# SonghuaHu-UMD/MultiSTGraph

Hardware: AMD Instinct MI355X
Metric: forward node-steps/s (B*T*N per second), MultiATGCN.predict (higher is better)
Workload: dtype f32; 1 GPU; Baltimore 403-node, in=24h out=24h, batch=64/GPU, multi+unidirection K=5; nodes=403, per_gpu_batch=64, global_batch=64, in_steps=24, out_steps=24, parallelism=batch shards, no data-path collective (dp1), layer_wavefront_streams=True

## Files before the change

multistgraph_amd/csrc/matgcn_kernels.hip:

```cpp
#include <hip/hip_runtime.h>
#include <stdint.h>

#include "matgcn_internal.h"

typedef __attribute__((ext_vector_type(16))) float f32x16;
typedef unsigned int u32x4 __attribute__((ext_vector_type(4)));
typedef __attribute__((ext_vector_type(4))) float f32x4;
#define MFMA16(a, b, c) __builtin_amdgcn_mfma_f32_16x16x4f32((a), (b), (c), 0, 0, 0)

#define MFMA32(a, b, c) __builtin_amdgcn_mfma_f32_32x32x2f32((a), (b), (c), 0, 0, 0)

__device__ __forceinline__ float sigmoid_f(float x) { return 1.0f / (1.0f + expf(-x)); }

__device__ __forceinline__ int acc_row(int r, int half) { return (r & 3) + 8 * (r >> 2) + 4 * half; }

__global__ __launch_bounds__(256) void k_adaptive_adj(const float* __restrict__ e1, const float* __restrict__ e2,
                                                      int rank, int bidir, int N, float* __restrict__ plain, int ldP) {
  extern __shared__ float logits[];
  __shared__ float red[256];
  __shared__ float erow[64];
  const int n = blockIdx.x, tid = threadIdx.x;
  for (int r = tid; r < rank; r += 256) erow[r] = e1[(size_t)n * rank + r];
  __syncthreads();
  float mx = 0.f;
// ... 16 lines not shown
  }
  mx = red[0];
  __syncthreads();
  float sum = 0.f;
  for (int m = tid; m < N; m += 256) {
    const float e = expf(logits[m] - mx);
    logits[m] = e;
    sum += e;
  }
  red[tid] = sum;
  __syncthreads();
  for (int s = 128; s > 0; s >>= 1) {
    if (tid < s) red[tid] += red[tid + s];
    __syncthreads();
  }
  const float inv = 1.0f / red[0];
  for (int m = tid; m < N; m += 256) plain[(size_t)n * ldP + m] = logits[m] * inv;
}

__global__ __launch_bounds__(256) void k_static_transpose(const float* __restrict__ S, int N, int ldSrc,
                                                          float* __restrict__ St, int ldS, int col0,
                                                          float* __restrict__ plain, int ldP, int accumulate) {
  __shared__ float tile[32][33];
  const int bx = blockIdx.x * 32, by = blockIdx.y * 32;
  const int tx = threadIdx.x & 31, ty = threadIdx.x >> 5;
  for (int j = ty; j < 32; j += 8) {
    const int n = by + j, m = bx + tx;
    const float v = (n < N && m < N) ? S[(size_t)n * ldSrc + m] : 0.f;
    tile[j][tx] = v;
    if (plain && plain != S && n < N && m < N) plain[(size_t)n * ldP + m] = v;
  }
  __syncthreads();
  for (int j = ty; j < 32; j += 8) {
    const int m = bx + j, n = by + tx;
    if (m < N && n < N) {
      float* dst = &St[(size_t)m * ldS + col0 + n];
      *dst = accumulate ? *dst + tile[tx][j] : tile[tx][j];
    }
  }
}

__global__ __launch_bounds__(256) void k_cheb_combine(const float* __restrict__ prod, const float* __restrict__ prev2,
                                                      int prev2_is_identity, int N, int ldP, float* __restrict__ St,
                                                      int ldS, int col0, float* __restrict__ plain_out) {
  __shared__ float tile[32][33];
  const int bx = blockIdx.x * 32, by = blockIdx.y * 32;
  const int tx = threadIdx.x & 31, ty = threadIdx.x >> 5;
  for (int j = ty; j < 32; j += 8) {
    const int n = by + j, m = bx + tx;
    float v = 0.f;
    if (n < N && m < N) {
      const float p2 = prev2_is_identity ? (n == m ? 1.f : 0.f) : prev2[(size_t)n * ldP + m];
      v = 2.0f * prod[(size_t)n * ldP + m] - p2;
      plain_out[(size_t)n * ldP + m] = v;
    }
    tile[j][tx] = v;
  }
  __syncthreads();
  for (int j = ty; j < 32; j += 8) {
    const int m = bx + j, n = by + tx;
    if (m < N && n < N) St[(size_t)m * ldS + col0 + n] = tile[tx][j];
  }
}

__global__ __launch_bounds__(256) void k_stack_tight(const float* __restrict__ St, int ldS, int Np, int N, int Ks,
                                                     float* __restrict__ tight, int ldT) {
  const size_t idx = (size_t)blockIdx.x * 256 + threadIdx.x;
  if (idx >= (size_t)Np * ldT) return;
  const int m = (int)(idx / ldT), c = (int)(idx % ldT);
  const int k = c / N, n = c - k * N;
  tight[idx] = k < Ks ? St[(size_t)m * ldS + k * Np + n] : 0.f;
}

__device__ __forceinline__ void stack_tail_zero(float* __restrict__ St, int ldS, float* __restrict__ StT, int ldT,
                                                int Np, int N, int Ks, int block, int nBlocks, int tid, int nThreads) {
  const int s0 = Ks * Np, t0 = Ks * N, ws = ldS - s0, wt = ldT - t0;
  for (int m = block; m < Np; m += nBlocks) {
    for (int c = tid; c < ws; c += nThreads) St[(size_t)m * ldS + s0 + c] = 0.f;
    for (int c = tid; c < wt; c += nThreads) StT[(size_t)m * ldT + t0 + c] = 0.f;
  }
}

template <int ROWS>
__global__ __launch_bounds__(256 * ROWS) void k_adaptive_stack(const float* __restrict__ e1, const float* __restrict__ e2,
                                                               int rank, int bidir, int N, int Np, int Ks,
                                                               float* __restrict__ St, int ldS, float* __restrict__ StT,
                                                               int ldT, int tail) {
  extern __shared__ float logitsAll[];
  __shared__ float redAll[ROWS][256];
  __shared__ float erowAll[ROWS][64];
  __shared__ float invAll[ROWS];
  const int sub = threadIdx.x >> 8, tid = threadIdx.x & 255;
  const int n0 = blockIdx.x * ROWS, n = n0 + sub;
  const bool live = n < N;
  float* logits = logitsAll + (size_t)sub * N;
  float* red = redAll[sub];
  float* erow = erowAll[sub];
  if (live)
    for (int r = tid; r < rank; r += 256) erow[r] = e1[(size_t)n * rank + r];
  __syncthreads();
  float mx = 0.f;
  if (live)
    for (int m = tid; m < N; m += 256) {
      float s = 0.f;
      if (bidir) {
        for (int r = 0; r < rank; ++r) s = fmaf(erow[r], e1[(size_t)m * rank + r], s);
      } else {
        for (int r = 0; r < rank; ++r) s = fmaf(erow[r], e2[(size_t)r * N + m], s);
      }
      s = fmaxf(s, 0.f);
      logits[m] = s;
      mx = fmaxf(mx, s);
    }
  red[tid] = mx;
  __syncthreads();
  for (int s = 128; s > 0; s >>= 1) {
    if (tid < s) red[tid] = fmaxf(red[tid], red[tid + s]);
    __syncthreads();
  }
  mx = red[0];
  __syncthreads();
  float sum = 0.f;
  if (live)
    for (int m = tid; m < N; m += 256) {
      const float e = expf(logits[m] - mx);
      logits[m] = e;
      sum += e;
    }
  red[tid] = sum;
  __syncthreads();
  for (int s = 128; s > 0; s >>= 1) {
    if (tid < s) red[tid] += red[tid + s];
    __syncthreads();
  }
  if (tid == 0) invAll[sub] = 1.0f / red[0];
  __syncthreads();
  for (int m = threadIdx.x; m < Np; m += 256 * ROWS) {
    float v[ROWS];
#pragma unroll
    for (int j = 0; j < ROWS; ++j) v[j] = (m < N && n0 + j < N) ? logitsAll[(size_t)j * N + m] * invAll[j] : 0.f;
    float* ds = St + (size_t)m * ldS + n0;
    float* dt = StT + (size_t)m * ldT + n0;
    if (ROWS == 4) {
      *reinterpret_cast<float4*>(ds) = make_float4(v[0], v[1], v[2], v[3]);
      if (n0 + 4 <= N) *reinterpret_cast<float4*>(dt) = make_float4(v[0], v[1], v[2], v[3]);
      else
#pragma unroll
        for (int j = 0; j < ROWS; ++j) if (n0 + j < N) dt[j] = v[j];
    } else {
#pragma unroll
      for (int j = 0; j < ROWS; ++j) {
        ds[j] = v[j];
        if (n0 + j < N) dt[j] = v[j];
      }
    }
  }
  if (tail) stack_tail_zero(St, ldS, StT, ldT, Np, N, Ks, blockIdx.x, gridDim.x, threadIdx.x, 256 * ROWS);
}

struct StaticStackArgs {
  const float* S[4];
  int slot[4];
};
__global__ __launch_bounds__(256) void k_static_stack(StaticStackArgs a, int N, int Np, int Ks, float* __restrict__ St,
                                                      int ldS, float* __restrict__ StT, int ldT, int tail) {
  __shared__ float tile[32][33];
  const float* __restrict__ S = a.S[blockIdx.z];
  const int slot = a.slot[blockIdx.z];
  const int bx = blockIdx.x * 32, by = blockIdx.y * 32;
  const int tx = threadIdx.x & 31, ty = threadIdx.x >> 5;
  for (int j = ty; j < 32; j += 8) {
    const int n = by + j, m = bx + tx;
    tile[j][tx] = (n < N && m < N) ? S[(size_t)n * N + m] : 0.f;
  }
  __syncthreads();
  for (int j = ty; j < 32; j += 8) {
    const int m = bx + j, n = by + tx;
    if (m < Np && n < Np) {
      St[(size_t)m * ldS + slot * Np + n] = tile[tx][j];
      if (n < N) StT[(size_t)m * ldT + slot * N + n] = tile[tx][j];
    }
  }
  if (tail)
    stack_tail_zero(St, ldS, StT, ldT, Np, N, Ks, (int)((blockIdx.z * gridDim.y + blockIdx.y) * gridDim.x + blockIdx.x),
                    (int)(gridDim.x * gridDim.y * gridDim.z), threadIdx.x, 256);
}

#define PREP_NB 8

__device__ __forceinline__ float cheb_scalar(float s, int order) {
  float t0 = 1.f, t1 = s;
  for (int j = 2; j <= order; ++j) { const float t2 = 2.f * s * t1 - t0; t0 = t1; t1 = t2; }
  return t1;
}

template <int KIND>
__global__ __launch_bounds__(256) void k_prep_stream(PrepStream a) {
  const int nBase = blockIdx.y * PREP_NB;
  const int unit = blockIdx.x * 256 + threadIdx.x;
  const int OT = a.O >> 4;
  if (unit >= a.groups * OT * 64) return;
  const int lane = unit & 63, ct = (unit >> 6) % OT, g = (unit >> 6) / OT;
  const int o = 16 * ct + (lane & 15);
  int slot[4], chan[4];
#pragma unroll
  for (int s = 0; s < 4; ++s) {
    if (KIND == 0) {
      const int kk = 16 * g + 4 * (lane >> 4) + s;
      slot[s] = kk >> 6; chan[s] = a.iOfs + (kk & 63);
    } else if (KIND == 1) {
      const int kk = 16 * g + 4 * (lane >> 4) + s;
      const int nx = a.map.nKeep * a.C0;
      if (kk < nx) { slot[s] = kk / a.C0; chan[s] = kk - slot[s] * a.C0; }
      else { slot[s] = kk == nx ? -2 : -1; chan[s] = 0; }
    }
  }
  float gmax = -3.0e38f, gsum = 1.f;
  if (a.wg) {
    gsum = 0.f;
    for (int k = 0; k < a.map.KtotOrig; ++k) gmax = fmaxf(gmax, a.wg[k]);
    for (int k = 0; k < a.map.KtotOrig; ++k) gsum += expf(a.wg[k] - gmax);
  }
  auto gk = [&](int k) { return a.wg ? expf(a.wg[k] - gmax) / gsum : 1.f; };
  const size_t dstride = (size_t)a.map.KtotOrig * a.I * a.O;
  float acc[PREP_NB][4];
#pragma unroll
  for (int b = 0; b < PREP_NB; ++b)
#pragma unroll
    for (int s = 0; s < 4; ++s) acc[b][s] = 0.f;
  size_t rofs[4];
  float scale[4];
#pragma unroll
  for (int s = 0; s < 4; ++s) {
    rofs[s] = 0; scale[s] = 0.f;
    if (slot[s] >= 0) {
      const int k = a.map.keepK[slot[s]];
      rofs[s] = ((size_t)k * a.I + chan[s]) * a.O + o;
      scale[s] = gk(k);
    } else if (slot[s] == -2) {
      scale[s] = 1.f;
    }
  }
#pragma unroll 4
  for (int dd = 0; dd < a.d; ++dd) {
    float pv[4];
#pragma unroll
    for (int s = 0; s < 4; ++s) {
      float v = 0.f;
      if (slot[s] >= 0) v = a.wpool[(size_t)dd * dstride + rofs[s]];
      else if (slot[s] == -2) v = a.bpool[(size_t)dd * a.O + o];
      pv[s] = v * scale[s];
    }
#pragma unroll
    for (int b = 0; b < PREP_NB; ++b) {
      const float e = a.E[(size_t)min(nBase + b, a.N - 1) * a.d + dd];
#pragma unroll
      for (int s = 0; s < 4; ++s) acc[b][s] = fmaf(e, pv[s], acc[b][s]);
    }
  }
  const bool anyIdent = slot[0] == 0 || slot[1] == 0 || slot[2] == 0 || slot[3] == 0;
  if (anyIdent) {
    for (int q = 0; q < a.map.nDiag; ++q) {
      const int k = a.map.diagK[q];
      const float gq = gk(k);
      float part[PREP_NB][4];
#pragma unroll
      for (int b = 0; b < PREP_NB; ++b)
#pragma unroll
        for (int s = 0; s < 4; ++s) part[b][s] = 0.f;
      for (int dd = 0; dd < a.d; ++dd) {
        float pv[4];
#pragma unroll
        for (int s = 0; s < 4; ++s)
          pv[s] = slot[s] == 0 ? a.wpool[(size_t)dd * dstride + ((size_t)k * a.I + chan[s]) * a.O + o] : 0.f;
#pragma unroll
        for (int b = 0; b < PREP_NB; ++b) {
          const float e = a.E[(size_t)min(nBase + b, a.N - 1) * a.d + dd];
#pragma unroll
          for (int s = 0; s < 4; ++s) part[b][s] = fmaf(e, pv[s], part[b][s]);
        }
      }
#pragma unroll
      for (int b = 0; b < PREP_NB; ++b) {
        const int n = min(nBase + b, a.N - 1);
        const float t = gq * cheb_scalar(a.map.diagSrc[q][(size_t)n * (a.map.N + 1)], a.map.diagOrder[q]);
#pragma unroll
        for (int s = 0; s < 4; ++s) acc[b][s] = fmaf(t, part[b][s], acc[b][s]);
      }
    }
  }
  size_t frag;
  if (a.OTdst > 0) frag = ((size_t)(g * a.OTdst + a.otOfs + ct) * 64 + lane) * 4;
  else frag = (size_t)unit * 4;
#pragma unroll
  for (int b = 0; b < PREP_NB; ++b) {
    const int n = nBase + b;
    if (n < a.N)
      *reinterpret_cast<float4*>(a.out + (size_t)n * a.nodeStride + a.baseOfs + frag) =
          make_float4(acc[b][0], acc[b][1], acc[b][2], acc[b][3]);
  }
}

template <int DS>
__global__ __launch_bounds__(256) void k_prep_mfma(PrepStream a, int tilesPerBlock) {
  const int tid = threadIdx.x, lane = tid & 63, w = tid >> 6;
  const int OT = a.O >> 4;
  const int pair = blockIdx.x >> 1, half = blockIdx.x & 1;
  const int ct = pair % OT, g = pair / OT;
  const int r = lane & 15, ka = lane >> 4;
  float gmax = -3.0e38f, gsum = 1.f;
  if (a.wg) {
    gsum = 0.f;
    for (int k = 0; k < a.map.KtotOrig; ++k) gmax = fmaxf(gmax, a.wg[k]);
    for (int k = 0; k < a.map.KtotOrig; ++k) gsum += expf(a.wg[k] - gmax);
  }
  auto gk = [&](int k) { return a.wg ? expf(a.wg[k] - gmax) / gsum : 1.f; };
  const size_t dstride = (size_t)a.map.KtotOrig * a.I * a.O;
  float A[8][DS], Aq[8][DS];
  bool ident = false;
#pragma unroll
  for (int q8 = 0; q8 < 8; ++q8) {
    const int kq = 2 * half + (q8 >> 2), j = 4 * (q8 & 3) + (r >> 2), sr = r & 3;
    const int o = 16 * ct + j;
    int slot, chan;
    if (g < a.groups) {
      const int kk = 16 * g + 4 * kq + sr;
      slot = kk >> 6; chan = a.iOfs + (kk & 63);
    } else {
      const int kk = 16 * (g - a.groups) + 4 * kq + sr;
      const int nx = a.map.nKeep * a.C0;
      if (kk < nx) { slot = kk / a.C0; chan = kk - slot * a.C0; }
      else { slot = kk == nx ? -2 : -1; chan = 0; }
    }
    const float* src = a.wpool; size_t sstep = 0; float scale = 0.f;
    if (slot >= 0) {
      const int k = a.map.keepK[slot];
      src = a.wpool + ((size_t)k * a.I + chan) * a.O + o; sstep = dstride; scale = gk(k);
    } else if (slot == -2) {
      src = a.bpool + o; sstep = (size_t)a.O; scale = 1.f;
    }
    const bool id = slot == 0 && a.map.nDiag > 0;
    ident = ident || id;
    const float* srcq = id ? a.wpool + ((size_t)a.map.diagK[0] * a.I + chan) * a.O + o : a.wpool;
#pragma unroll
    for (int st = 0; st < DS; ++st) {
      const int dd = 4 * st + ka;
      const float v = src[(size_t)min(dd, a.d - 1) * sstep];
      A[q8][st] = (dd < a.d && slot != -1) ? v * scale : 0.f;
      const float vq = srcq[(size_t)min(dd, a.d - 1) * (id ? dstride : 0)];
      Aq[q8][st] = (dd < a.d && id) ? vq : 0.f;
    }
  }
  const bool anyIdent = __ballot(ident) != 0ull;
  const int nTiles = (a.N + 15) >> 4;
  const int tile0 = blockIdx.y * tilesPerBlock, tile1 = min(tile0 + tilesPerBlock, nTiles);
  const int nodeL = lane & 15, kb = lane >> 4;
  auto load_b = [&](int tile, float (&Bf)[DS]) {
    const float* e = a.E + (size_t)min(tile * 16 + nodeL, a.N - 1) * a.d;
#pragma unroll
    for (int st = 0; st < DS; ++st) {
      const int dd = 4 * st + kb;
      const float v = e[min(dd, a.d - 1)];
      Bf[st] = dd < a.d ? v : 0.f;
    }
  };
  float Bf[DS], Bn[DS];
  if (tile0 + w < tile1) load_b(tile0 + w, Bf);
  for (int tile = tile0 + w; tile < tile1; tile += 4) {
    load_b(min(tile + 4, tile1 - 1), Bn);
    const int n = tile * 16 + nodeL;
    f32x4 acc[8];
#pragma unroll
    for (int q8 = 0; q8 < 8; ++q8) acc[q8] = f32x4{0.f, 0.f, 0.f, 0.f};
#pragma unroll
    for (int st = 0; st < DS; ++st)
#pragma unroll
      for (int q8 = 0; q8 < 8; ++q8) acc[q8] = MFMA16(A[q8][st], Bf[st], acc[q8]);
    if (anyIdent) {
      const int nc = min(n, a.N - 1);
      for (int q = 0; q < a.map.nDiag; ++q) {
        f32x4 part[8];
#pragma unroll
        for (int q8 = 0; q8 < 8; ++q8) part[q8] = f32x4{0.f, 0.f, 0.f, 0.f};
        if (q == 0) {
#pragma unroll
          for (int st = 0; st < DS; ++st)
#pragma unroll
            for (int q8 = 0; q8 < 8; ++q8) part[q8] = MFMA16(Aq[q8][st], Bf[st], part[q8]);
        } else {
          const int k = a.map.diagK[q];
#pragma unroll
          for (int q8 = 0; q8 < 8; ++q8) {
            const int kq = 2 * half + (q8 >> 2), j = 4 * (q8 & 3) + (r >> 2), sr = r & 3;
            int slot, chan;
            if (g < a.groups) { const int kk = 16 * g + 4 * kq + sr; slot = kk >> 6; chan = a.iOfs + (kk & 63); }
            else {
              const int kk = 16 * (g - a.groups) + 4 * kq + sr;
              if (kk < a.map.nKeep * a.C0) { slot = kk / a.C0; chan = kk - slot * a.C0; } else { slot = -1; chan = 0; }
            }
#pragma unroll
            for (int st = 0; st < DS; ++st) {
              const int dd = 4 * st + ka;
              const float v = a.wpool[(size_t)min(dd, a.d - 1) * dstride + ((size_t)k * a.I + chan) * a.O + 16 * ct + j];
              part[q8] = MFMA16((dd < a.d && slot == 0) ? v : 0.f, Bf[st], part[q8]);
            }
          }
        }
        const float t = gk(a.map.diagK[q]) *
                        cheb_scalar(a.map.diagSrc[q][(size_t)nc * (a.map.N + 1)], a.map.diagOrder[q]);
#pragma unroll
        for (int q8 = 0; q8 < 8; ++q8)
#pragma unroll
          for (int e = 0; e < 4; ++e) acc[q8][e] = fmaf(t, part[q8][e], acc[q8][e]);
      }
    }
    if (n < a.N) {
      float* dst = a.out + (size_t)n * a.nodeStride + a.baseOfs;
#pragma unroll
      for (int q8 = 0; q8 < 8; ++q8) {
        const int kq = 2 * half + (q8 >> 2), j = 4 * (q8 & 3) + kb;
        const size_t frag = ((size_t)(a.OTdst > 0 ? g * a.OTdst + a.otOfs + ct : g * OT + ct) * 64 + kq * 16 + j) * 4;
        *reinterpret_cast<float4*>(dst + frag) = make_float4(acc[q8][0], acc[q8][1], acc[q8][2], acc[q8][3]);
      }
    }
#pragma unroll
    for (int st = 0; st < DS; ++st) Bf[st] = Bn[st];
  }
}

__global__ __launch_bounds__(256) void k_prep_bias(const float* __restrict__ E, const float* __restrict__ bpool, int d,
                                                   int O, int N, float* __restrict__ out, int ldo, int colOfs) {
  const int idx = blockIdx.x * 256 + threadIdx.x;
  if (idx >= N * O) return;
  const int n = idx / O, o = idx - n * O;
  float s = 0.f;
  for (int dd = 0; dd < d; ++dd) s = fmaf(E[(size_t)n * d + dd], bpool[(size_t)dd * O + o], s);
  out[(size_t)n * ldo + colOfs + o] = s;
}

__device__ __forceinline__ void prep_linear(const float* __restrict__ W, int I, int O, int C, int Cpad, int rows, int OT,
                                            float* __restrict__ out, int unit) {
  const int units = (rows >> 3) * OT * 64;
  if (unit >= units) return;
  const int lane = unit & 63, ot = (unit >> 6) % OT, jg = (unit >> 6) / OT;
  const int o = ot * 32 + (lane & 31);
  float v[4];
#pragma unroll
  for (int q = 0; q < 4; ++q) {
    const int j = jg * 8 + 4 * (lane >> 5) + q;
    int in = -1;
    if (j < Cpad) { if (j < C) in = j; } else { in = C + (j - Cpad); }
    v[q] = (in >= 0 && in < I && o < O) ? W[(size_t)o * I + in] : 0.f;
  }
  *reinterpret_cast<float4*>(out + (size_t)unit * 4) = make_float4(v[0], v[1], v[2], v[3]);
}

__global__ __launch_bounds__(256) void k_pack_rows(const float* __restrict__ src, float* __restrict__ dst, int rows,
                                                   int N, int Np, int C) {
  const size_t idx = (size_t)blockIdx.x * 256 + threadIdx.x;
  const size_t total = (size_t)rows * Np * C;
  if (idx >= total) return;
  const int c = idx % C;
  const int n = (idx / C) % Np;
  const size_t r = idx / ((size_t)C * Np);
  dst[idx] = (src && n < N) ? src[(r * N + n) * C + c] : 0.f;
}

__global__ __launch_bounds__(256) void k_unpack_rows(const float* __restrict__ src, float* __restrict__ dst, int rows,
                                                     int N, int Np, int C) {
  const size_t idx = (size_t)blockIdx.x * 256 + threadIdx.x;
  const size_t total = (size_t)rows * N * C;
  if (idx >= total) return;
  const int c = idx % C;
  const int n = (idx / C) % N;
  const size_t r = idx / ((size_t)C * N);
  dst[idx] = src[(r * Np + n) * C + c];
}

__global__ __launch_bounds__(256) void k_pack_seq_tm(const float* __restrict__ src, float* __restrict__ dst, int B,
                                                     int T, int N, int Np, int C) {
  const size_t idx = (size_t)blockIdx.x * 256 + threadIdx.x;
  const size_t total = (size_t)T * B * Np * C;
  if (idx >= total) return;
  const int c = idx % C;
  const int n = (idx / C) % Np;
  const int b = (idx / ((size_t)C * Np)) % B;
  const int t = idx / ((size_t)C * Np * B);
  dst[idx] = (n < N) ? src[(((size_t)b * T + t) * N + n) * C + c] : 0.f;
}

__global__ __launch_bounds__(256) void k_unpack_seq_tm(const float* __restrict__ src, float* __restrict__ dst, int B,
                                                       int T, int N, int Np, int C) {
  const size_t idx = (size_t)blockIdx.x * 256 + threadIdx.x;
  const size_t total = (size_t)B * T * N * C;
  if (idx >= total) return;
  const int c = idx % C;
  const int n = (idx / C) % N;
  const int t = (idx / ((size_t)C * N)) % T;
  const int b = idx / ((size_t)C * N * T);
  dst[idx] = src[(((size_t)t * B + b) * Np + n) * C + c];
}

__global__ __launch_bounds__(256) void k_zero_pad_rows(float* __restrict__ buf, int rows, int N, int Np, int C) {
  const int per = (Np - N) * C;
  const size_t idx = (size_t)blockIdx.x * 256 + threadIdx.x;
  if (idx >= (size_t)rows * per) return;
  const size_t r = idx / per;
  const int q = idx - r * per;
  buf[(r * Np + N) * C + q] = 0.f;
}

struct PadRowBufs { float* p[8]; };
__global__ __launch_bounds__(256) void k_zero_pad_rows_multi(PadRowBufs bufs, int rows, int N, int Np, int C) {
  const int per4 = (Np - N) * C / 4;
  const size_t idx = (size_t)blockIdx.x * 256 + threadIdx.x;
  if (idx >= (size_t)rows * per4) return;
  const size_t r = idx / per4;
  const int q = (int)(idx - r * per4);
  *reinterpret_cast<float4*>(bufs.p[blockIdx.y] + (r * Np + N) * C + 4 * q) = make_float4(0.f, 0.f, 0.f, 0.f);
}

__device__ unsigned long long g_series_violations = 0;
__device__ __forceinline__ size_t series_row(long row, long steps) {
  if (row < 0 || row >= steps) {
    atomicAdd(&g_series_violations, 1ull);
    row = row < 0 ? 0 : steps - 1;
  }
  return (size_t)row;
}

__global__ __launch_bounds__(256) void k_fuse_heads(FuseArgs a) {
  const size_t idx = (size_t)blockIdx.x * 256 + threadIdx.x;
  const size_t total = (size_t)a.B * a.T * a.Np;
  if (idx >= total) return;
  const int n = idx % a.Np;
  const int t = (idx / a.Np) % a.T;
  const int b = idx / ((size_t)a.Np * a.T);
  if (n >= a.N) {
    float* pad = a.x0 + idx * a.C0;
    for (int c = 0; c < a.C0; ++c) pad[c] = 0.f;
    return;
  }
  float gmax = -3.0e38f, gsum = 0.f;
  for (int h = 0; h < a.nTs; ++h) gmax = fmaxf(gmax, a.tsg[h]);
  for (int h = 0; h < a.nTs; ++h) gsum += expf(a.tsg[h] - gmax);
  auto xrow = [&](int step) -> const float* {
    const size_t r = a.labelStart ? series_row((long)a.labelStart[b] + a.rel[step], a.seriesSteps)
                                  : (size_t)b * a.xSteps + step;
    return a.X + (r * a.N + n) * a.F;
  };
  float* dst = a.x0 + (((size_t)b * a.T + t) * a.Np + n) * a.C0;
  for (int c = 0; c < a.od; ++c) {
    float acc = 0.f;
    for (int h = 0; h < a.nHeads; ++h) {
      const float g = expf(a.tsg[h] - gmax) / gsum;
      const float xv = xrow(a.headBegin[h] + t)[a.startDim + c];
      const float wv = a.ts[h][((size_t)t * a.N + n) * a.od + c];
      acc += g * xv * wv;
    }
    dst[c] = acc;
  }
  for (int j = 0; j < a.C0 - a.od; ++j)
    dst[a.od + j] = xrow(t)[a.extSrc[j]];
}

__global__ __launch_bounds__(256) void k_x0_to_matrix(const float* __restrict__ x0p, float* __restrict__ X0m, int rows,
                                                      int Np, int C0, int ld) {
  const size_t idx = (size_t)blockIdx.x * 256 + threadIdx.x;
  const size_t total = (size_t)Np * ld;
  if (idx >= total) return;
  const int col = idx % ld;
  const int m = idx / ld;
  float v = 0.f;
  if (col < rows * C0) {
    const int row = col / C0, c = col - row * C0;
    v = x0p[((size_t)row * Np + m) * C0 + c];
  }
  X0m[idx] = v;
}

__global__ __launch_bounds__(256) void k_build_xa0(const float* __restrict__ X0m, const float* __restrict__ MX0,
                                                   float* __restrict__ XA0, int B, int T, int N, int Np, int C0,
                                                   int Ks, int Kx, int ld, int bChunk, int tChunk) {
  extern __shared__ float xs[];
  const int n = blockIdx.x, b0 = blockIdx.y * bChunk, t0 = blockIdx.z * tChunk;
  const int nb = min(bChunk, B - b0), nt = min(tChunk, T - t0);
  const int run = nt * C0, perK = nb * run;
  for (int i = threadIdx.x; i < (Ks + 1) * perK; i += 256) {
    const int k = i / perK, r = i - k * perK;
    const int bb = r / run, q = r - bb * run;
    const float* src = k == 0 ? X0m + (size_t)n * ld : MX0 + ((size_t)(k - 1) * Np + n) * ld;
    xs[i] = src[((size_t)(b0 + bb) * T + t0) * C0 + q];
  }
  __syncthreads();
  const int nx = (Ks + 1) * C0, kx4 = Kx >> 2, perT = nb * kx4;
  for (int i = threadIdx.x; i < nt * perT; i += 256) {
    const int tt = i / perT, r = i - tt * perT;
    const int bb = r / kx4, j0 = 4 * (r - bb * kx4);
    float v[4];
#pragma unroll
    for (int e = 0; e < 4; ++e) {
      const int j = j0 + e;
      v[e] = 0.f;
      if (j < nx) {
        const int k = j / C0, c = j - k * C0;
        v[e] = xs[(k * nb + bb) * run + tt * C0 + c];
      } else if (j == nx) v[e] = 1.0f;
    }
    float* dst = XA0 + (((size_t)(t0 + tt) * N + n) * B + b0) * Kx + 4 * (size_t)r;
    *reinterpret_cast<float4*>(dst) = make_float4(v[0], v[1], v[2], v[3]);
  }
}

struct StateInitArgs {
  float* zhx[4];
  float* hx[4];
  float* h0dst[4];
  const float* h0[4];
  float* seq[4];
};
__global__ __launch_bounds__(256) void k_state_init(StateInitArgs a, int B, int rowsSeq, int N, int Np) {
  const int l = blockIdx.y;
  const size_t idx = (size_t)blockIdx.x * 256 + threadIdx.x;
  const size_t state4 = (size_t)B * Np * 16;
  const float4 zero = make_float4(0.f, 0.f, 0.f, 0.f);
  if (idx < state4) {
    const int c4 = (int)(idx & 15);
    const int n = (int)((idx >> 4) % Np);
    const size_t r = (idx >> 4) / Np;
    float4 v = zero;
    if (a.h0[l] && n < N) {
      const float* src = a.h0[l] + (r * N + n) * 64 + 4 * c4;
      v = make_float4(src[0], src[1], src[2], src[3]);
    }
    reinterpret_cast<float4*>(a.zhx[l])[idx] = zero;
    reinterpret_cast<float4*>(a.hx[l])[idx] = v;
    if (a.h0dst[l]) reinterpret_cast<float4*>(a.h0dst[l])[idx] = v;
    return;
  }
  const int per4 = (Np - N) * 16;
  const size_t q = idx - state4;
  if (q >= (size_t)rowsSeq * per4) return;
  const size_t r = q / per4;
  const int e = (int)(q - r * per4);
  *reinterpret_cast<float4*>(a.seq[l] + (r * Np + N) * 64 + 4 * e) = zero;
}

constexpr int MIX_FLUSH_TILES = 16;

__device__ __forceinline__ void mix_tile_order(int id, int nColUnits, int nRowTiles, int& rowTile, int& colUnit) {
  if ((nColUnits & 7) == 0) {
    const int xcd = id & 7, j = id >> 3, cpx = nColUnits >> 3;
    rowTile = j % nRowTiles;
    colUnit = xcd * cpx + j / nRowTiles;
  } else {
    rowTile = id % nRowTiles;
    colUnit = id / nRowTiles;
  }
}

template <int ROLE, bool FLUSH = false>
__global__ __launch_bounds__(256) void k_mix(MixArgs a) {
  __shared__ __attribute__((aligned(16))) float As[2][16 * 64];
  __shared__ __attribute__((aligned(16))) float Bs[2][16 * 64];
  int colTile, rowTile;
  mix_tile_order(blockIdx.x, a.nColTiles, a.nRowTiles, rowTile, colTile);
  const int row0 = rowTile * 64;
  const int tid = threadIdx.x, lane = tid & 63, w = tid >> 6;
  const int wr = w >> 1, wc = w & 1, j = lane & 15, kq = lane >> 4;
  const int kk = tid >> 4, sg = tid & 15;
  const int part = blockIdx.y;
  const float* ap = a.St + (size_t)part * a.aPartStride + (size_t)kk * a.ldS + row0 + sg * 4;
  const float* bp = a.X + (size_t)part * a.xPartStride + (size_t)colTile * a.xTileStride + (size_t)kk * a.ldX + sg * 4;
  const int stPos = kk * 64 + (((sg + 4 * (kk & 3)) & 15) << 2);
  const int last = a.nK - 1;
  auto ldA = [&](int t) { return *reinterpret_cast<const float4*>(ap + (size_t)min(t, last) * 16 * a.ldS); };
  auto ldB = [&](int t) { return *reinterpret_cast<const float4*>(bp + (size_t)min(t, last) * 16 * a.ldX); };
  float4 ra0, rb0, ra1, rb1;
  {
    const float4 a0 = ldA(0), b0 = ldB(0);
    __builtin_amdgcn_sched_barrier(0);
    ra0 = ldA(1); rb0 = ldB(1); ra1 = ldA(2); rb1 = ldB(2);
    __builtin_amdgcn_sched_barrier(0);
    *reinterpret_cast<float4*>(&As[0][stPos]) = a0;
    *reinterpret_cast<float4*>(&Bs[0][stPos]) = b0;
  }
  __syncthreads();
  f32x4 acc[2][2], tot[FLUSH ? 2 : 1][2];
#pragma unroll
  for (int p = 0; p < 2; ++p)
#pragma unroll
    for (int q = 0; q < 2; ++q) {
      acc[p][q] = f32x4{0.f, 0.f, 0.f, 0.f};
      if constexpr (FLUSH) tot[p][q] = f32x4{0.f, 0.f, 0.f, 0.f};
    }
  const int rotA0 = (wr * 32 + j + 16 * kq) & 63, rotA1 = (wr * 32 + 16 + j + 16 * kq) & 63;
  const int rotB0 = (wc * 32 + j + 16 * kq) & 63, rotB1 = (wc * 32 + 16 + j + 16 * kq) & 63;
  auto mma = [&](int cur) {
    const float* A = &As[cur][kq * 64];
    const float* Bm = &Bs[cur][kq * 64];
#pragma unroll
    for (int s = 0; s < 4; ++s) {
      const float a0 = A[s * 256 + rotA0], a1 = A[s * 256 + rotA1];
      const float b0 = Bm[s * 256 + rotB0], b1 = Bm[s * 256 + rotB1];
      acc[0][0] = MFMA16(a0, b0, acc[0][0]);
      acc[0][1] = MFMA16(a0, b1, acc[0][1]);
      acc[1][0] = MFMA16(a1, b0, acc[1][0]);
      acc[1][1] = MFMA16(a1, b1, acc[1][1]);
    }
  };
  for (int it = 0; it < a.nK; it += 2) {
    mma(0);
    *reinterpret_cast<float4*>(&As[1][stPos]) = ra0;
    *reinterpret_cast<float4*>(&Bs[1][stPos]) = rb0;
    ra0 = ldA(it + 3); rb0 = ldB(it + 3);
    __syncthreads();
    if (it + 1 < a.nK) {
      mma(1);
      *reinterpret_cast<float4*>(&As[0][stPos]) = ra1;
      *reinterpret_cast<float4*>(&Bs[0][stPos]) = rb1;
      ra1 = ldA(it + 4); rb1 = ldB(it + 4);
      __syncthreads();
    }
    if constexpr (FLUSH) {
      if (((it + 2) & (MIX_FLUSH_TILES - 1)) == 0) {
#pragma unroll
        for (int p = 0; p < 2; ++p)
#pragma unroll
          for (int q = 0; q < 2; ++q) {
// ... 1011 lines not shown
```

Baseline: 98.10 million node-steps/s.

## Restructure prep MFMA kernel with LDS-staged stores and batched B/coefficient loads

Reworks the per-node weight generation MFMA kernel. Gate softmax weights and kept-slot indices now come from a shared-memory table instead of being recomputed per lane. Four node tiles of B fragments and diagonal Chebyshev coefficients are staged in LDS per wave. Output fragments go through a swizzled LDS buffer and are written with 128-bit buffer stores, giving coalesced contiguous row writes. Launch bounds also request two blocks per SM for small DS. The cost is extra LDS traffic and wave barriers, plus higher LDS footprint that may limit occupancy.

```diff
diff --git a/multistgraph_amd/csrc/matgcn_kernels.hip b/multistgraph_amd/csrc/matgcn_kernels.hip
--- a/multistgraph_amd/csrc/matgcn_kernels.hip
+++ b/multistgraph_amd/csrc/matgcn_kernels.hip
@@ -342,22 +342,29 @@
 }
 
 template <int DS>
-__global__ __launch_bounds__(256) void k_prep_mfma(PrepStream a, int tilesPerBlock) {
+__global__ __launch_bounds__(256, DS <= 5 ? 2 : 1) void k_prep_mfma(PrepStream a, int tilesPerBlock) {
   const int tid = threadIdx.x, lane = tid & 63, w = tid >> 6;
   const int OT = a.O >> 4;
   const int pair = blockIdx.x >> 1, half = blockIdx.x & 1;
   const int ct = pair % OT, g = pair / OT;
   const int r = lane & 15, ka = lane >> 4;
-  float gmax = -3.0e38f, gsum = 1.f;
-  if (a.wg) {
-    gsum = 0.f;
-    for (int k = 0; k < a.map.KtotOrig; ++k) gmax = fmaxf(gmax, a.wg[k]);
-    for (int k = 0; k < a.map.KtotOrig; ++k) gsum += expf(a.wg[k] - gmax);
-  }
-  auto gk = [&](int k) { return a.wg ? expf(a.wg[k] - gmax) / gsum : 1.f; };
+  __shared__ float gtab[MATGCN_MAX_STACK];
+  __shared__ int keepTab[MATGCN_MAX_STACK];
+  if (tid < MATGCN_MAX_STACK) {
+    float gv = 1.f;
+    if (a.wg && tid < a.map.KtotOrig) {
+      float gmax = -3.0e38f, gsum = 0.f;
+      for (int k = 0; k < a.map.KtotOrig; ++k) gmax = fmaxf(gmax, a.wg[k]);
+      for (int k = 0; k < a.map.KtotOrig; ++k) gsum += expf(a.wg[k] - gmax);
+      gv = expf(a.wg[tid] - gmax) / gsum;
+    }
+    gtab[tid] = gv;
+    keepTab[tid] = a.map.keepK[tid];
+  }
+  __syncthreads();
   const size_t dstride = (size_t)a.map.KtotOrig * a.I * a.O;
-  float A[8][DS], Aq[8][DS];
-  bool ident = false;
+  float A[8][DS], Aq[8][DS], scale[8];
+  unsigned live = 0u, idm = 0u;
 #pragma unroll
   for (int q8 = 0; q8 < 8; ++q8) {
     const int kq = 2 * half + (q8 >> 2), j = 4 * (q8 & 3) + (r >> 2), sr = r & 3;
@@ -372,25 +379,31 @@
       if (kk < nx) { slot = kk / a.C0; chan = kk - slot * a.C0; }
       else { slot = kk == nx ? -2 : -1; chan = 0; }
     }
-    const float* src = a.wpool; size_t sstep = 0; float scale = 0.f;
-    if (slot >= 0) {
-      const int k = a.map.keepK[slot];
-      src = a.wpool + ((size_t)k * a.I + chan) * a.O + o; sstep = dstride; scale = gk(k);
-    } else if (slot == -2) {
-      src = a.bpool + o; sstep = (size_t)a.O; scale = 1.f;
-    }
+    const int k = keepTab[max(slot, 0)];
+    const bool row = slot >= 0, bias = slot == -2;
+    const float* src = row ? a.wpool + ((size_t)k * a.I + chan) * a.O + o : bias ? a.bpool + o : a.wpool;
+    const size_t sstep = row ? dstride : bias ? (size_t)a.O : 0;
+    scale[q8] = row ? gtab[k] : bias ? 1.f : 0.f;
     const bool id = slot == 0 && a.map.nDiag > 0;
-    ident = ident || id;
     const float* srcq = id ? a.wpool + ((size_t)a.map.diagK[0] * a.I + chan) * a.O + o : a.wpool;
+    live |= (slot != -1 ? 1u : 0u) << q8;
+    idm |= (id ? 1u : 0u) << q8;
 #pragma unroll
     for (int st = 0; st < DS; ++st) {
       const int dd = 4 * st + ka;
-      const float v = src[(size_t)min(dd, a.d - 1) * sstep];
-      A[q8][st] = (dd < a.d && slot != -1) ? v * scale : 0.f;
-      const float vq = srcq[(size_t)min(dd, a.d - 1) * (id ? dstride : 0)];
-      Aq[q8][st] = (dd < a.d && id) ? vq : 0.f;
-    }
-  }
+      A[q8][st] = src[(size_t)min(dd, a.d - 1) * sstep];
+      Aq[q8][st] = srcq[(size_t)min(dd, a.d - 1) * (id ? dstride : 0)];
+    }
+  }
+#pragma unroll
+  for (int q8 = 0; q8 < 8; ++q8)
+#pragma unroll
+    for (int st = 0; st < DS; ++st) {
+      const int dd = 4 * st + ka;
+      A[q8][st] = (dd < a.d && (live >> q8 & 1u)) ? A[q8][st] * scale[q8] : 0.f;
+      Aq[q8][st] = (dd < a.d && (idm >> q8 & 1u)) ? Aq[q8][st] : 0.f;
+    }
+  const bool ident = idm != 0u;
   const bool anyIdent = __ballot(ident) != 0ull;
   const int nTiles = (a.N + 15) >> 4;
   const int tile0 = blockIdx.y * tilesPerBlock, tile1 = min(tile0 + tilesPerBlock, nTiles);
@@ -404,67 +417,106 @@
       Bf[st] = dd < a.d ? v : 0.f;
     }
   };
-  float Bf[DS], Bn[DS];
-  if (tile0 + w < tile1) load_b(tile0 + w, Bf);
-  for (int tile = tile0 + w; tile < tile1; tile += 4) {
-    load_b(min(tile + 4, tile1 - 1), Bn);
-    const int n = tile * 16 + nodeL;
-    f32x4 acc[8];
-#pragma unroll
-    for (int q8 = 0; q8 < 8; ++q8) acc[q8] = f32x4{0.f, 0.f, 0.f, 0.f};
-#pragma unroll
-    for (int st = 0; st < DS; ++st)
-#pragma unroll
-      for (int q8 = 0; q8 < 8; ++q8) acc[q8] = MFMA16(A[q8][st], Bf[st], acc[q8]);
+  __shared__ f32x4 rows[4][16 * 32];
+  f32x4* const my = rows[w];
+  float* const dstRow = a.out + a.baseOfs +
+                        ((size_t)(a.OTdst > 0 ? g * a.OTdst + a.otOfs + ct : g * OT + ct) * 64 + 2 * half * 16) * 4;
+  auto store_rows = [&](int tile) {
+    const int f = lane & 31, hi = lane >> 5;
+    const f32x4* const src = my + hi * 32;
+    const int t = __builtin_amdgcn_readfirstlane(tile);
+    const int live = min(16, a.N - 16 * t);
+    const auto rsrc = __builtin_amdgcn_make_buffer_rsrc(dstRow + (size_t)t * 16 * a.nodeStride, 0,
+                                                        (int)(((size_t)(live - 1) * a.nodeStride + 128) * 4), 0x00020000);
+    f32x4 v[8];
+#pragma unroll
+    for (int i = 0; i < 8; ++i) v[i] = src[2 * i * 32 + ((f & 16) | ((f ^ (2 * i + hi)) & 15))];
+#pragma unroll
+    for (int i = 0; i < 8; ++i) {
+      const u32x4 bits = {__float_as_uint(v[i][0]), __float_as_uint(v[i][1]), __float_as_uint(v[i][2]),
+                          __float_as_uint(v[i][3])};
+      const size_t off = (size_t)(2 * i + hi) * a.nodeStride + 4 * f;
+      __builtin_amdgcn_raw_buffer_store_b128(bits, rsrc, (int)(off * 4), 0, 16);
+    }
+  };
+  __shared__ float bst[4][4][DS][64];
+  __shared__ float tst[4][4][MATGCN_MAX_STACK][16];
+  for (int c0 = tile0 + w; c0 < tile1; c0 += 16) {
+#pragma unroll
+    for (int ts = 0; ts < 4; ++ts) {
+      float Bt[DS];
+      load_b(min(c0 + 4 * ts, nTiles - 1), Bt);
+#pragma unroll
+      for (int st = 0; st < DS; ++st) bst[w][ts][st][lane] = Bt[st];
+    }
     if (anyIdent) {
-      const int nc = min(n, a.N - 1);
-      for (int q = 0; q < a.map.nDiag; ++q) {
-        f32x4 part[8];
-#pragma unroll
-        for (int q8 = 0; q8 < 8; ++q8) part[q8] = f32x4{0.f, 0.f, 0.f, 0.f};
-        if (q == 0) {
-#pragma unroll
-          for (int st = 0; st < DS; ++st)
-#pragma unroll
-            for (int q8 = 0; q8 < 8; ++q8) part[q8] = MFMA16(Aq[q8][st], Bf[st], part[q8]);
-        } else {
-          const int k = a.map.diagK[q];
-#pragma unroll
-          for (int q8 = 0; q8 < 8; ++q8) {
-            const int kq = 2 * half + (q8 >> 2), j = 4 * (q8 & 3) + (r >> 2), sr = r & 3;
-            int slot, chan;
-            if (g < a.groups) { const int kk = 16 * g + 4 * kq + sr; slot = kk >> 6; chan = a.iOfs + (kk & 63); }
-            else {
-              const int kk = 16 * (g - a.groups) + 4 * kq + sr;
-              if (kk < a.map.nKeep * a.C0) { slot = kk / a.C0; chan = kk - slot * a.C0; } else { slot = -1; chan = 0; }
-            }
-#pragma unroll
-            for (int st = 0; st < DS; ++st) {
-              const int dd = 4 * st + ka;
-              const float v = a.wpool[(size_t)min(dd, a.d - 1) * dstride + ((size_t)k * a.I + chan) * a.O + 16 * ct + j];
-              part[q8] = MFMA16((dd < a.d && slot == 0) ? v : 0.f, Bf[st], part[q8]);
+      const int nc = min(min(c0 + 4 * kb, nTiles - 1) * 16 + nodeL, a.N - 1);
+      for (int q = 0; q < a.map.nDiag; ++q)
+        tst[w][kb][q][nodeL] = gtab[a.map.diagK[q]] *
+                               cheb_scalar(a.map.diagSrc[q][(size_t)nc * (a.map.N + 1)], a.map.diagOrder[q]);
+    }
+    __builtin_amdgcn_fence(__ATOMIC_ACQ_REL, "wavefront");
+    __builtin_amdgcn_wave_barrier();
+#pragma unroll 1
+    for (int ts = 0; ts < 4 && c0 + 4 * ts < tile1; ++ts) {
+      const int tile = c0 + 4 * ts;
+      float Bf[DS];
+#pragma unroll
+      for (int st = 0; st < DS; ++st) Bf[st] = bst[w][ts][st][lane];
+      f32x4 acc[8];
+#pragma unroll
+      for (int q8 = 0; q8 < 8; ++q8) acc[q8] = f32x4{0.f, 0.f, 0.f, 0.f};
+#pragma unroll
+      for (int st = 0; st < DS; ++st)
+#pragma unroll
+        for (int q8 = 0; q8 < 8; ++q8) acc[q8] = MFMA16(A[q8][st], Bf[st], acc[q8]);
+      if (anyIdent) {
+        for (int q = 0; q < a.map.nDiag; ++q) {
+          f32x4 part[8];
+#pragma unroll
+          for (int q8 = 0; q8 < 8; ++q8) part[q8] = f32x4{0.f, 0.f, 0.f, 0.f};
+          if (q == 0) {
+#pragma unroll
+            for (int st = 0; st < DS; ++st)
+#pragma unroll
+              for (int q8 = 0; q8 < 8; ++q8) part[q8] = MFMA16(Aq[q8][st], Bf[st], part[q8]);
+          } else {
+            const int k = a.map.diagK[q];
+#pragma unroll
+            for (int q8 = 0; q8 < 8; ++q8) {
+              const int kq = 2 * half + (q8 >> 2), j = 4 * (q8 & 3) + (r >> 2), sr = r & 3;
+              int slot, chan;
+              if (g < a.groups) { const int kk = 16 * g + 4 * kq + sr; slot = kk >> 6; chan = a.iOfs + (kk & 63); }
+              else {
+                const int kk = 16 * (g - a.groups) + 4 * kq + sr;
+                if (kk < a.map.nKeep * a.C0) { slot = kk / a.C0; chan = kk - slot * a.C0; } else { slot = -1; chan = 0; }
+              }
+#pragma unroll
+              for (int st = 0; st < DS; ++st) {
+                const int dd = 4 * st + ka;
+                const float v = a.wpool[(size_t)min(dd, a.d - 1) * dstride + ((size_t)k * a.I + chan) * a.O + 16 * ct + j];
+                part[q8] = MFMA16((dd < a.d && slot == 0) ? v : 0.f, Bf[st], part[q8]);
+              }
             }
           }
+          const float t = tst[w][ts][q][nodeL];
+#pragma unroll
+          for (int q8 = 0; q8 < 8; ++q8)
+#pragma unroll
+            for (int e = 0; e < 4; ++e) acc[q8][e] = fmaf(t, part[q8][e], acc[q8][e]);
         }
-        const float t = gk(a.map.diagK[q]) *
-                        cheb_scalar(a.map.diagSrc[q][(size_t)nc * (a.map.N + 1)], a.map.diagOrder[q]);
-#pragma unroll
-        for (int q8 = 0; q8 < 8; ++q8)
-#pragma unroll
-          for (int e = 0; e < 4; ++e) acc[q8][e] = fmaf(t, part[q8][e], acc[q8][e]);
       }
-    }
-    if (n < a.N) {
-      float* dst = a.out + (size_t)n * a.nodeStride + a.baseOfs;
 #pragma unroll
       for (int q8 = 0; q8 < 8; ++q8) {
-        const int kq = 2 * half + (q8 >> 2), j = 4 * (q8 & 3) + kb;
-        const size_t frag = ((size_t)(a.OTdst > 0 ? g * a.OTdst + a.otOfs + ct : g * OT + ct) * 64 + kq * 16 + j) * 4;
-        *reinterpret_cast<float4*>(dst + frag) = make_float4(acc[q8][0], acc[q8][1], acc[q8][2], acc[q8][3]);
+        const int f = 16 * (q8 >> 2) + 4 * (q8 & 3) + kb;
+        my[nodeL * 32 + ((f & 16) | ((f ^ nodeL) & 15))] = acc[q8];
       }
-    }
-#pragma unroll
-    for (int st = 0; st < DS; ++st) Bf[st] = Bn[st];
+      __builtin_amdgcn_fence(__ATOMIC_ACQ_REL, "wavefront");
+      __builtin_amdgcn_wave_barrier();
+      store_rows(tile);
+      __builtin_amdgcn_fence(__ATOMIC_ACQ_REL, "wavefront");
+      __builtin_amdgcn_wave_barrier();
+    }
   }
 }
 
```

New measurement: 98.45 million node-steps/s, median of 6. Within noise of the previous version (+0.4%).
